# MyNiuuu/MOFA-Video

Measured on AMD Instinct MI355X. Metric: denoised frames/sec, 25f 576x1024 SVD+MOFA, 25 steps, higher is better.
Workload: dtype f16; 1 GPU; MOFA-Video-Traj, 25-frame 576x1024, 25 denoise steps + temporal VAE decode (chunk 8), single trajectory hint, SVD-XT UNet + MOFA-Adapter, CFG 1->3, seeded random weights in the reference checkpoint layout; num_frames=25, height=576, width=1024, num_inference_steps=25, decode_chunk_size=8, parallelism=1 GPU, graph_steps=False, output_finite=True

## Files before the change

### mofa_video_amd/csrc/igemm8.hip

```cpp
#include "igemm_common.h"
#include "igemm_pipe.h"

namespace {

constexpr int WM = 2, WN = 4, MI = 4, NJ = 2;
constexpr int TBM = WM * MI * 32, TBN = WN * NJ * 32;
constexpr int BKS = 64, RB = 128;
constexpr int SXB = TBM * RB, STB = SXB + TBN * RB;
constexpr int SCRATCH0 = 2 * STB, SCRATCH_WAVE = 4096;
constexpr int LDS_BYTES = SCRATCH0 + 8 * SCRATCH_WAVE;
constexpr int LOOKAHEAD_OPS = 8;

struct Cursor {
    int local;
    int ikc, ksw, ky, kx;
    int gx0, gx1;
    unsigned xo0, xo1;
    unsigned wo0, wo1, wo2, wo3;
};

template <int EPI, int VAR = 0>
__global__ __launch_bounds__(512, 2) void igemm8_f16_kernel(const mofa_igemm_args a, const int tilesN, const int ntiles,
                                                            const Aux aux) {
    constexpr bool GEGLU = (EPI & EPI_GEGLU) != 0, R1 = (EPI & EPI_R1) != 0, R2 = (EPI & EPI_R2) != 0,
                   RV = (EPI & EPI_RV) != 0;
    extern __shared__ __attribute__((aligned(16))) char smem[];
    TileWalk walk;
    walk.init(ntiles);
    if (walk.local >= walk.count) return;
    const int tid = threadIdx.x, lane = tid & 63;
    const int wave = __builtin_amdgcn_readfirstlane(tid >> 6);
    const int grp = wave >> 2;
    const int wm = wave / WN, wn = wave - wm * WN;
    const int l31 = lane & 31, lh = lane >> 5;

    const int taps = igemm_taps(a);
    const int kpt = a.Cin / BKS, nk = taps * kpt;
    const size_t Ktot = (size_t)taps * a.Cin;

    auto swz_bytes = [&](int l, int q) __attribute__((always_inline)) { return (((l & 7) ^ (4 * q + (l >> 4))) * 16); };
    auto x_row = [&](int h, int q, int hr0) __attribute__((always_inline)) { const int hr = hr0 + 8 * q; return (hr >> 6) * 128 + h * 64 + (hr & 63); };
    auto w_row = [&](int h, int q, int hr0) __attribute__((always_inline)) { const int hr = hr0 + 8 * q; return (hr >> 5) * 64 + h * 32 + (hr & 31); };
    const TapGeo tg(a);
    const BufRsrc rsx = buf_rsrc(aux.xbase, aux.x_bytes), rsw = buf_rsrc(a.w, aux.w_bytes);
    const LdsDma16 bglds16;
    auto cur_setup = [&](Cursor& c, const int h, const bool with_w) __attribute__((always_inline)) {
        const bool live = c.local < walk.count;
        const int tile = walk.start + (live ? c.local : 0);
        const int tm = fdiv(tile, aux.tiles_n), tn = tile - tm * tilesN;
        const int l = lane_now(lane), hr_l = 16 * wave + (l >> 3);
        const int g0 = pack_geo(a, aux, tm * TBM + x_row(h, 0, hr_l)), g1 = pack_geo(a, aux, tm * TBM + x_row(h, 1, hr_l));
        c.gx0 = live ? g0 : -1;
        c.gx1 = live ? g1 : -1;
        if (with_w) {
            auto w_off = [&](int hq) __attribute__((always_inline)) {
                int n = tn * TBN + w_row(hq >> 1, hq & 1, hr_l);
                n = n < a.N ? n : a.N - 1;
                const unsigned o = (unsigned)n * (unsigned)(Ktot * 2) + swz_bytes(l, hq & 1);
                return live ? o : XO_INVALID;
            };
            c.wo0 = w_off(0); c.wo1 = w_off(1); c.wo2 = w_off(2); c.wo3 = w_off(3);
        }
        c.ikc = 0; c.ksw = 0; c.ky = 0; c.kx = 0;
    };
    auto issue_x = [&](Cursor& c, const int h, const int bo) __attribute__((always_inline)) {
        if (c.ikc == 0) {
            const int l = lane_now(lane);
            c.xo0 = tap_src(a, aux, tg, c.gx0, c.ky, c.kx, swz_bytes(l, 0));
            c.xo1 = tap_src(a, aux, tg, c.gx1, c.ky, c.kx, swz_bytes(l, 1));
        }
        bglds16(rsx, c.xo0, c.ikc * (BKS * 2), smem + bo + x_row(h, 0, 16 * wave) * RB);
        bglds16(rsx, c.xo1, c.ikc * (BKS * 2), smem + bo + x_row(h, 1, 16 * wave) * RB);
    };
    auto issue_w = [&](Cursor& c, const int bo) __attribute__((always_inline)) {
        bglds16(rsw, c.wo0, c.ksw * (BKS * 2), smem + bo + SXB + w_row(0, 0, 16 * wave) * RB);
        bglds16(rsw, c.wo1, c.ksw * (BKS * 2), smem + bo + SXB + w_row(0, 1, 16 * wave) * RB);
        bglds16(rsw, c.wo2, c.ksw * (BKS * 2), smem + bo + SXB + w_row(1, 0, 16 * wave) * RB);
        bglds16(rsw, c.wo3, c.ksw * (BKS * 2), smem + bo + SXB + w_row(1, 1, 16 * wave) * RB);
    };
    auto advance = [&](Cursor& c, const int h, const bool with_w) __attribute__((always_inline)) {
        tap_advance(c, a, kpt, tg.ks);
        if (c.ksw == nk) { c.local += walk.stride; cur_setup(c, h, with_w); }
    };

    int xa[4], wa[4];
    {
        const int fsw = (l31 >> 1) & 7;
#pragma unroll
        for (int kk = 0; kk < 4; ++kk) {
            const int slot = ((kk * 2 + lh) ^ fsw) * 16;
            xa[kk] = (wm * MI * 32 + l31) * RB + slot;
            wa[kk] = SXB + (wn * NJ * 32 + l31) * RB + slot;
        }
    }

    char* scr = smem + SCRATCH0 + wave * SCRATCH_WAVE;
    const BufRsrc rsb = buf_rsrc(a.bias, a.bias ? (unsigned)a.N * 4u : 0u);
    auto bias_prefetch = [&](int nw, int slot = 0) __attribute__((always_inline)) {
        __builtin_amdgcn_raw_ptr_buffer_load_lds(rsb, (__attribute__((address_space(3))) void*)(scr + slot * 256), 4,
                                                 (unsigned)(nw + lane_now(lane)) * 4u, 0, 0, 0);
    };
    constexpr bool BIAS_INIT = GEGLU;

    Cursor ca, cb;
    ca.local = cb.local = walk.local;
    cur_setup(ca, 0, true);
    cur_setup(cb, 1, false);
    if constexpr (BIAS_INIT) {
        const int tile0 = walk.start + walk.local;
        bias_prefetch((tile0 - fdiv(tile0, aux.tiles_n) * tilesN) * TBN + wn * NJ * 32, 0);
    }
    issue_x(ca, 0, 0); issue_w(ca, 0); advance(ca, 0, true);
    issue_x(cb, 1, 0); advance(cb, 1, false);
    issue_x(ca, 0, STB); issue_w(ca, STB); advance(ca, 0, true);
    wait_vmcnt_only<LOOKAHEAD_OPS>();
    __builtin_amdgcn_s_barrier();

    f32x16 acc[MI][NJ];
    f16x8 xf[2][4], wf[2][4];
    unsigned long long tr[13] = {0, 0, 0, 0, 0, 0, 0, 0, 0, 0, 0, 0, 0}, tr_t = 0;
    if (VAR & 64) tr_t = __builtin_readcyclecounter();
    if (VAR & 32) {
#pragma unroll
        for (int kk = 0; kk < 4; ++kk) {
            xf[0][kk] = *(const f16x8*)(smem + xa[kk]);
            xf[1][kk] = *(const f16x8*)(smem + xa[kk] + 32 * RB);
            wf[0][kk] = *(const f16x8*)(smem + wa[kk]);
            wf[1][kk] = *(const f16x8*)(smem + wa[kk] + 32 * RB);
        }
    }
    auto stamp = [&](int k) __attribute__((always_inline)) {
        if (VAR & 64) { const unsigned long long t = __builtin_readcyclecounter(); tr[k] += t - tr_t; tr_t = t; }
    };
    auto phase = [&](auto pc, const int bo, const int bn) __attribute__((always_inline)) {
        constexpr int P = decltype(pc)::v;
        auto reads = [&]() __attribute__((always_inline)) {
            if (VAR & 32) return;
#pragma unroll
            for (int il = 0; il < 2; ++il)
#pragma unroll
                for (int kk = 0; kk < 4; ++kk)
                    xf[il][kk] = *(const f16x8*)(smem + xa[kk] + ((P == 2 ? 2 : 0) + il) * 32 * RB);
            if constexpr (P == 1) {
#pragma unroll
                for (int j = 0; j < 2; ++j)
#pragma unroll
                    for (int kk = 0; kk < 4; ++kk) wf[j][kk] = *(const f16x8*)(smem + wa[kk] + j * 32 * RB);
            }
        };
        auto issues = [&]() __attribute__((always_inline)) {
            if (VAR & 16) return;
            if constexpr (P == 1) issue_x(cb, 1, bn);
            if constexpr (P == 2) { issue_x(ca, 0, bo); issue_w(ca, bo); }
        };
        if (VAR & 4) { issues(); __builtin_amdgcn_sched_barrier(0); reads(); }
        else { reads(); __builtin_amdgcn_sched_barrier(0); issues(); }
        if constexpr (P == 1) advance(cb, 1, false);
        if constexpr (P == 2) advance(ca, 0, true);
        if (!(VAR & 8)) wait_vmcnt<LOOKAHEAD_OPS>(); else wait_lds();
        __builtin_amdgcn_sched_barrier(0);
        __builtin_amdgcn_s_barrier();
        __builtin_amdgcn_sched_barrier(0);
        stamp(3 * (P - 1));
        if (!(VAR & 2)) __builtin_amdgcn_s_setprio(1);
#pragma unroll
        for (int kk = 0; kk < 4; ++kk)
#pragma unroll
            for (int il = 0; il < 2; ++il)
#pragma unroll
                for (int j = 0; j < 2; ++j) {
                    constexpr int I0 = (P == 2) ? 2 : 0;
                    acc[I0 + il][j] = __builtin_amdgcn_mfma_f32_32x32x16_f16(wf[j][kk], xf[il][kk], acc[I0 + il][j], 0, 0, 0);
                }
        if (!(VAR & 2)) __builtin_amdgcn_s_setprio(0);
        stamp(3 * (P - 1) + 1);
        __builtin_amdgcn_sched_barrier(0);
        __builtin_amdgcn_s_barrier();
        __builtin_amdgcn_sched_barrier(0);
        stamp(3 * (P - 1) + 2);
    };

    auto epilogue_light = [&](auto ac, auto un, f32x16 (&acc)[MI][NJ], const int mw, const int nw, const int idx_u) __attribute__((always_inline)) {
        constexpr bool UNI = decltype(un)::v != 0;
        constexpr bool SACC1 = GEGLU && UNI;
        const int lane_e = RV ? lane_now(lane) : lane;
        const int lane = lane_e, l31 = lane & 31, lh = lane >> 5;
        f16* out = (f16*)a.out;
        float saccv = a.s_acc;
        asm volatile("" : "+v"(saccv));
        f32x4 bv[NJ][4];
        if (!BIAS_INIT && (!RV || UNI)) {
#pragma unroll
            for (int j = 0; j < NJ; ++j)
#pragma unroll
                for (int g = 0; g < 4; ++g) bv[j][g] = *(const f32x4*)(scr + (32 * j + 8 * g + 4 * lh) * 4);
        }
        const int nout = GEGLU ? a.N / 2 : a.N;
        int rv_div = a.rv_div, rv_mod_in = a.rv_mod_in, rv_mod_out = a.rv_mod_out;
        asm volatile("" : "+s"(rv_div), "+s"(rv_mod_in), "+s"(rv_mod_out));
        f32x4 rv[NJ][4];
        auto rv_load = [&](int i, f32x4 (&rv)[NJ][4]) __attribute__((always_inline)) {
            int m = mw + 32 * i + l31;
            m = m < a.M ? m : a.M - 1;
            const int idx = UNI ? idx_u : ((m / rv_div) * a.rv_mul + (m % rv_mod_in)) % rv_mod_out;
            const float* rvp = a.rowvec + (size_t)idx * a.N;
#pragma unroll
            for (int j = 0; j < NJ; ++j)
#pragma unroll
                for (int g = 0; g < 4; ++g) {
                    int n = nw + 32 * j + 8 * g + 4 * lh;
                    n = n + 4 <= a.N ? n : 0;
                    rv[j][g] = *(const f32x4*)(rvp + n);
                    if (!UNI && a.bias) rv[j][g] += *(const f32x4*)(a.bias + n);
                }
        };
        if (RV) rv_load(0, rv);
        if (RV && UNI) {
#pragma unroll
            for (int j = 0; j < NJ; ++j)
#pragma unroll
                for (int g = 0; g < 4; ++g) bv[j][g] += rv[j][g];
        }
        auto store_pair = [&](f16x4 g0, f16x4 g1, int m, int n0) __attribute__((always_inline)) {
            typedef unsigned u32x2 __attribute__((ext_vector_type(2)));
            typedef unsigned u32x4 __attribute__((ext_vector_type(4)));
            u32x2 a2 = __builtin_bit_cast(u32x2, g0), b2 = __builtin_bit_cast(u32x2, g1);
            const auto rx = __builtin_amdgcn_permlane32_swap(a2[0], b2[0], false, false);
            const auto ry = __builtin_amdgcn_permlane32_swap(a2[1], b2[1], false, false);
            const u32x4 v = {rx[0], ry[0], rx[1], ry[1]};
            const int n = n0 + 8 * lh;
            if (m < a.M && n + 8 <= nout) *(u32x4*)(out + (size_t)m * a.ldo + n) = v;
        };
#pragma unroll
        for (int i = 0; i < MI; ++i) {
            const int m = mw + 32 * i + l31;
            if constexpr (GEGLU) {
                f16x4 o[4];
#pragma unroll
                for (int g = 0; g < 4; ++g)
#pragma unroll
                    for (int e = 0; e < 4; ++e) {
                        const float val = acc[i][g >> 1][4 * (g & 1) + e];
                        const float gate = acc[i][g >> 1][8 + 4 * (g & 1) + e];
                        if constexpr (SACC1) o[g][e] = (f16)(val * (gate * gelu_phi_f(gate)));
                        else o[g][e] = (f16)(saccv * val * gelu_erf_f(saccv * gate));
                    }
                store_pair(o[0], o[1], m, nw / 2);
                store_pair(o[2], o[3], m, nw / 2 + 16);
            } else {
#pragma unroll
                for (int j = 0; j < NJ; ++j)
#pragma unroll
                    for (int g = 0; g < 4; ++g) {
                        f16x4 o;
#pragma unroll
                        for (int e = 0; e < 4; ++e) {
                            const float v = acc[i][j][4 * g + e] + (RV && !UNI ? rv[j][g][e] : bv[j][g][e]);
                            o[e] = (f16)act_apply(ac, saccv * v);
                        }
                        *(f16x4*)(scr + h16_off(l31 * 128, l31, 8 * j + 2 * g + lh)) = o;
                    }
                if (RV && !UNI && i + 1 < MI) rv_load(i + 1, rv);
#pragma unroll
                for (int p = 0; p < 4; ++p) {
                    const H16Piece r = h16_row<4 * NJ>(scr, RowLines128{}, lane, p);
                    const int mr = mw + 32 * i + r.row, n = nw + 8 * r.blk;
                    if (mr < a.M && n + 8 <= nout) *(f16x8*)(out + (size_t)mr * a.ldo + n) = r.v;
                }
            }
        }
    };
    auto epilogue_residual = [&](auto un, f32x16 (&acc)[MI][NJ], const int mw, const int nw, const int idx_u) __attribute__((always_inline)) {
        constexpr bool UNI = decltype(un)::v != 0;
        constexpr int STEPS = MI * NJ;
        constexpr int REGS = (R1 ? 8 : 0) + (R2 ? 8 : 0) + (RV && !UNI ? 16 : 0);
        constexpr int D0 = REGS <= 8 ? 8 : (REGS <= 16 ? 4 : (REGS <= 24 ? 2 : 1));
        constexpr int D = RV && UNI ? (REGS <= 8 ? 4 : 2) : (RV ? 1 : D0);
        const int lane_e = RV ? lane_now(lane) : lane;
        const int lane = lane_e, l31 = lane & 31, lh = lane >> 5;
        f16* out = (f16*)a.out;
        const f16* r1 = (const f16*)a.r1;
        const f16* r2 = (const f16*)a.r2;
        float s1v = a.s1, s2v = a.s2, saccv = a.s_acc;
        asm volatile("" : "+v"(s1v), "+v"(s2v), "+v"(saccv));
        int rv_div = a.rv_div, rv_mod_in = a.rv_mod_in, rv_mod_out = a.rv_mod_out;
        asm volatile("" : "+s"(rv_div), "+s"(rv_mod_in), "+s"(rv_mod_out));
        const int piece = lane & 3;
        struct StepLoads { f16x8 t1[2], t2[2]; f32x4 rv0[2], rv1[2]; };
        StepLoads L[D];
        auto step_loads = [&](int st, StepLoads& l) __attribute__((always_inline)) {
            const int i = st / NJ, j = st % NJ;
            const int n = nw + 32 * j + 8 * piece;
            const int nc = n + 8 <= a.N ? n : 0;
#pragma unroll
            for (int p = 0; p < 2; ++p) {
                int m = mw + 32 * i + 16 * p + (lane >> 2);
                m = m < a.M ? m : a.M - 1;
                if (R1) l.t1[p] = *(const f16x8*)(r1 + (size_t)m * a.ldr1 + nc);
                if (R2) l.t2[p] = *(const f16x8*)(r2 + (size_t)m * a.ldr2 + nc);
                if (RV && !UNI) {
                    const int idx = ((m / rv_div) * a.rv_mul + (m % rv_mod_in)) % rv_mod_out;
                    const float* q = a.rowvec + (size_t)idx * a.N + nc;
                    l.rv0[p] = *(const f32x4*)q;
                    l.rv1[p] = *(const f32x4*)(q + 4);
                }
            }
        };
        f32x4 rvu[NJ][2];
        if (RV && UNI) {
#pragma unroll
            for (int j = 0; j < NJ; ++j) {
                const int n = nw + 32 * j + 8 * piece;
                const float* q = a.rowvec + (size_t)idx_u * a.N + (n + 8 <= a.N ? n : 0);
                rvu[j][0] = *(const f32x4*)q;
                rvu[j][1] = *(const f32x4*)(q + 4);
            }
        }
#pragma unroll
        for (int st = 0; st < D && st < STEPS; ++st) step_loads(st, L[st]);
        f32x4 bv[NJ][2];
#pragma unroll
        for (int j = 0; j < NJ; ++j) {
            bv[j][0] = *(const f32x4*)(scr + (32 * j + 8 * piece) * 4);
            bv[j][1] = *(const f32x4*)(scr + (32 * j + 8 * piece + 4) * 4);
            if (RV && UNI) { bv[j][0] += rvu[j][0]; bv[j][1] += rvu[j][1]; }
        }
#pragma unroll
        for (int st = 0; st < STEPS; ++st) {
            const int i = st / NJ, j = st % NJ;
            StepLoads& l = L[st % D];
#pragma unroll
            for (int g = 0; g < 4; ++g) {
                f32x4 v;
#pragma unroll
                for (int e = 0; e < 4; ++e) v[e] = acc[i][j][4 * g + e];
                *(f32x4*)(scr + f32_off(l31 * 128, l31, 2 * g + lh)) = v;
            }
            const int n = nw + 32 * j + 8 * piece;
#pragma unroll
            for (int p = 0; p < 2; ++p) {
                const int row = 16 * p + (lane >> 2);
                const f32x4 v0 = *(const f32x4*)(scr + f32_off(row * 128, row, 2 * piece));
                const f32x4 v1 = *(const f32x4*)(scr + f32_off(row * 128, row, 2 * piece + 1));
                f16x8 o;
#pragma unroll
                for (int e = 0; e < 4; ++e) {
                    float x0 = v0[e] + bv[j][0][e], x1 = v1[e] + bv[j][1][e];
                    if (RV && !UNI) { x0 += l.rv0[p][e]; x1 += l.rv1[p][e]; }
                    x0 *= saccv; x1 *= saccv;
                    if (R1 || R2) { x0 = (float)(f16)x0; x1 = (float)(f16)x1; }
                    if (R1) { x0 += s1v * (float)l.t1[p][e]; x1 += s1v * (float)l.t1[p][4 + e]; }
                    if (R2) { x0 += s2v * (float)l.t2[p][e]; x1 += s2v * (float)l.t2[p][4 + e]; }
                    o[e] = (f16)x0; o[4 + e] = (f16)x1;
                }
                const int m = mw + 32 * i + row;
                if (m < a.M && n + 8 <= a.N) *(f16x8*)(out + (size_t)m * a.ldo + n) = o;
            }
            if (st + D < STEPS) step_loads(st + D, L[st % D]);
        }
    };

    int gt = 0;
    int bslot = 0;
    for (int cl = walk.local; cl < walk.count; cl += walk.stride, bslot ^= 1) {
        const int tile = walk.start + cl;
        const int tm = fdiv(tile, aux.tiles_n), tn = tile - tm * tilesN;
        if (VAR & 64) { stamp(9); tr[12] += nk; }
        if constexpr (BIAS_INIT) {
            int tn2 = tn;
            if (cl + walk.stride < walk.count) {
                const int tile2 = walk.start + cl + walk.stride;
                tn2 = tile2 - fdiv(tile2, aux.tiles_n) * tilesN;
            }
            bias_prefetch(tn2 * TBN + wn * NJ * 32, bslot ^ 1);
            const int lh_e = lane_now(lane) >> 5;
#pragma unroll
            for (int j = 0; j < NJ; ++j)
#pragma unroll
                for (int g = 0; g < 4; ++g) {
                    const f32x4 b = *(const f32x4*)(scr + bslot * 256 + (32 * j + 8 * g + 4 * lh_e) * 4);
#pragma unroll
                    for (int i = 0; i < MI; ++i)
#pragma unroll
                        for (int e = 0; e < 4; ++e) acc[i][j][4 * g + e] = b[e];
                }
        } else {
#pragma unroll
            for (int i = 0; i < MI; ++i)
#pragma unroll
                for (int j = 0; j < NJ; ++j)
#pragma unroll
                    for (int r = 0; r < 16; ++r) acc[i][j][r] = 0.0f;

            bias_prefetch(tn * TBN + wn * NJ * 32);
        }
        if (!(VAR & 1) && grp == 1) __builtin_amdgcn_s_barrier();
        for (int kt = 0; kt < nk; ++kt, ++gt) {
            const int bo = (gt & 1) * STB, bn = STB - bo;
            phase(IC<1>{}, bo, bn);
            phase(IC<2>{}, bo, bn);
#pragma unroll
            for (int kk = 0; kk < 4; ++kk) { xa[kk] ^= STB; wa[kk] ^= STB; }
        }
        if (!(VAR & 1) && grp == 0) __builtin_amdgcn_s_barrier();
        stamp(6);

        const int mw = tm * TBM + wm * MI * 32;
        const int nw = tn * TBN + wn * NJ * 32;
        int idx_u = -1;
        if constexpr (RV) idx_u = rowvec_uniform_idx<32 * MI>(a, mw);
        if constexpr (R1 || R2) {
            if (RV && idx_u >= 0) epilogue_residual(IC<1>{}, acc, mw, nw, idx_u);
            else epilogue_residual(IC<0>{}, acc, mw, nw, 0);
        } else if constexpr (GEGLU) {
            if (a.s_acc == 1.0f) epilogue_light(IC<MOFA_ACT_NONE>{}, IC<1>{}, acc, mw, nw, 0);
            else epilogue_light(IC<MOFA_ACT_NONE>{}, IC<0>{}, acc, mw, nw, 0);
        } else if constexpr (RV) {
            if (idx_u >= 0) epilogue_light(IC<MOFA_ACT_NONE>{}, IC<1>{}, acc, mw, nw, idx_u);
            else epilogue_light(IC<MOFA_ACT_NONE>{}, IC<0>{}, acc, mw, nw, 0);
        } else {
            if (a.act == MOFA_ACT_NONE) epilogue_light(IC<MOFA_ACT_NONE>{}, IC<0>{}, acc, mw, nw, 0);
            else if (a.act == MOFA_ACT_SILU) epilogue_light(IC<MOFA_ACT_SILU>{}, IC<0>{}, acc, mw, nw, 0);
            else if (a.act == MOFA_ACT_RELU) epilogue_light(IC<MOFA_ACT_RELU>{}, IC<0>{}, acc, mw, nw, 0);
            else epilogue_light(IC<MOFA_ACT_GELU>{}, IC<0>{}, acc, mw, nw, 0);
        }
        if (VAR & 64) { stamp(7); tr[8] += 1; }
    }
    wait_vmcnt_only<0>();
    if ((VAR & 64) && aux.trace && (tid & 255) == 0) {
#pragma unroll
        for (int k = 0; k < 13; ++k) aux.trace[((size_t)blockIdx.x * 2 + grp) * 16 + k] = tr[k];
    }
}

typedef void (*igemm8_kern_t)(const mofa_igemm_args, const int, const int, const Aux);

}

static const igemm8_kern_t k_igemm8[9] = {igemm8_f16_kernel<0>, igemm8_f16_kernel<1>, igemm8_f16_kernel<2>,
                                           igemm8_f16_kernel<3>, igemm8_f16_kernel<4>, igemm8_f16_kernel<5>,
                                           igemm8_f16_kernel<6>, igemm8_f16_kernel<7>, igemm8_f16_kernel<8>};


#ifdef MOFA_PROBE
static int s_probe_var = 0;
static unsigned long long* s_probe_trace = nullptr;
static const int k_probe_vars[] = {1, 2, 4, 8, 16, 32, 48, 64};
static const igemm8_kern_t k_trace_kern[9] = {nullptr, igemm8_f16_kernel<1, 64>, nullptr, nullptr, igemm8_f16_kernel<4, 64>, nullptr, nullptr,
                                               nullptr, igemm8_f16_kernel<8, 64>};
static const igemm8_kern_t k_probe_kern[] = {
    igemm8_f16_kernel<0, 1>, igemm8_f16_kernel<0, 2>, igemm8_f16_kernel<0, 4>, igemm8_f16_kernel<0, 8>,
    igemm8_f16_kernel<0, 16>, igemm8_f16_kernel<0, 32>, igemm8_f16_kernel<0, 48>, igemm8_f16_kernel<0, 64>};
extern "C" int mofa_igemm8_set_probe(int var, void* trace) {
    s_probe_var = var;
    s_probe_trace = (unsigned long long*)trace;
    return 0;
}
#endif

int igemm8_init() {
    if (mofa_lds_optin(k_igemm8, LDS_BYTES) != MOFA_OK) return MOFA_ELAUNCH;
#ifdef MOFA_PROBE
    if (mofa_lds_optin(k_probe_kern, LDS_BYTES) != MOFA_OK || mofa_lds_optin(k_trace_kern, LDS_BYTES) != MOFA_OK) return MOFA_ELAUNCH;
#endif
    return MOFA_OK;
}

int igemm8_launch(const mofa_igemm_args* a, int kind, int n_cu, hipStream_t stream) {
    const int taps = igemm_taps(*a);
    if (!igemm_pipe_eligible(a, kind, (long long)taps * a->Cin)) return 1;
    const int tilesM = cdiv(a->M, TBM), tilesN = cdiv(a->N, TBN);
    const long long nt = (long long)tilesM * tilesN;
    if (nt > 0x7fffffffLL) return MOFA_EINVAL;
    Aux aux = igemm_pipe_aux(a, taps, tilesN);
    igemm8_kern_t kern = k_igemm8[kind];
#ifdef MOFA_PROBE
    aux.trace = s_probe_trace;
    if (kind == 0 && s_probe_var)
        for (size_t i = 0; i < sizeof(k_probe_vars) / sizeof(int); ++i)
            if (k_probe_vars[i] == s_probe_var) kern = k_probe_kern[i];
    if (s_probe_var == 64 && k_trace_kern[kind]) kern = k_trace_kern[kind];
#endif
    hipLaunchKernelGGL(kern, dim3(igemm_grid(nt, n_cu)), dim3(512), LDS_BYTES, stream, *a, tilesN, (int)nt, aux);
    MOFA_CHECK_LAUNCH();
    return MOFA_OK;
}
```

Baseline: 4.251 frames/s.

## Switch igemm8 inner MFMA from 32x32x16 to 16x16x32 with epilogue permute

Replaces each 32x32x16 MFMA with four 16x16x32 MFMAs per accumulator tile. It also reworks the LDS fragment addressing and swizzle so each lane reads 16-row fragments over two k-halves. After the K loop, permlane16_swap shuffles the accumulators back into the 32x32 register layout the existing epilogues expect, and the bias initialisation is adapted to match. The aim is higher MFMA throughput or lower issue latency with the smaller instruction. In exchange the MFMA instruction count rises, and extra per-element vector shuffles are added around each MFMA and in the epilogue.

```diff
diff --git a/mofa_video_amd/csrc/igemm8.hip b/mofa_video_amd/csrc/igemm8.hip
--- a/mofa_video_amd/csrc/igemm8.hip
+++ b/mofa_video_amd/csrc/igemm8.hip
@@ -83,14 +83,14 @@
         if (c.ksw == nk) { c.local += walk.stride; cur_setup(c, h, with_w); }
     };
 
-    int xa[4], wa[4];
+    int xa[2], wa[2];
     {
-        const int fsw = (l31 >> 1) & 7;
-#pragma unroll
-        for (int kk = 0; kk < 4; ++kk) {
-            const int slot = ((kk * 2 + lh) ^ fsw) * 16;
-            xa[kk] = (wm * MI * 32 + l31) * RB + slot;
-            wa[kk] = SXB + (wn * NJ * 32 + l31) * RB + slot;
+        const int r = lane & 15, c = lane >> 4;
+        const int rw = 8 * ((r >> 2) & 1) + 4 * (r >> 3) + (r & 3);
+#pragma unroll
+        for (int ks = 0; ks < 2; ++ks) {
+            xa[ks] = (wm * MI * 32 + r) * RB + ((4 * ks + c) ^ ((r >> 1) & 7)) * 16;
+            wa[ks] = SXB + (wn * NJ * 32 + rw) * RB + ((4 * ks + c) ^ ((rw >> 1) & 7)) * 16;
         }
     }
 
@@ -122,12 +122,12 @@
     if (VAR & 64) tr_t = __builtin_readcyclecounter();
     if (VAR & 32) {
 #pragma unroll
-        for (int kk = 0; kk < 4; ++kk) {
-            xf[0][kk] = *(const f16x8*)(smem + xa[kk]);
-            xf[1][kk] = *(const f16x8*)(smem + xa[kk] + 32 * RB);
-            wf[0][kk] = *(const f16x8*)(smem + wa[kk]);
-            wf[1][kk] = *(const f16x8*)(smem + wa[kk] + 32 * RB);
-        }
+        for (int ks = 0; ks < 2; ++ks)
+#pragma unroll
+            for (int f = 0; f < 4; ++f) {
+                xf[ks][f] = *(const f16x8*)(smem + xa[ks] + f * 16 * RB);
+                wf[ks][f] = *(const f16x8*)(smem + wa[ks] + f * 16 * RB);
+            }
     }
     auto stamp = [&](int k) __attribute__((always_inline)) {
         if (VAR & 64) { const unsigned long long t = __builtin_readcyclecounter(); tr[k] += t - tr_t; tr_t = t; }
@@ -137,15 +137,15 @@
         auto reads = [&]() __attribute__((always_inline)) {
             if (VAR & 32) return;
 #pragma unroll
-            for (int il = 0; il < 2; ++il)
-#pragma unroll
-                for (int kk = 0; kk < 4; ++kk)
-                    xf[il][kk] = *(const f16x8*)(smem + xa[kk] + ((P == 2 ? 2 : 0) + il) * 32 * RB);
+            for (int ks = 0; ks < 2; ++ks)
+#pragma unroll
+                for (int f = 0; f < 4; ++f)
+                    xf[ks][f] = *(const f16x8*)(smem + xa[ks] + ((P == 2 ? 4 : 0) + f) * 16 * RB);
             if constexpr (P == 1) {
 #pragma unroll
-                for (int j = 0; j < 2; ++j)
-#pragma unroll
-                    for (int kk = 0; kk < 4; ++kk) wf[j][kk] = *(const f16x8*)(smem + wa[kk] + j * 32 * RB);
+                for (int ks = 0; ks < 2; ++ks)
+#pragma unroll
+                    for (int f = 0; f < 4; ++f) wf[ks][f] = *(const f16x8*)(smem + wa[ks] + f * 16 * RB);
             }
         };
         auto issues = [&]() __attribute__((always_inline)) {
@@ -164,20 +164,49 @@
         stamp(3 * (P - 1));
         if (!(VAR & 2)) __builtin_amdgcn_s_setprio(1);
 #pragma unroll
-        for (int kk = 0; kk < 4; ++kk)
+        for (int ks = 0; ks < 2; ++ks)
 #pragma unroll
             for (int il = 0; il < 2; ++il)
 #pragma unroll
-                for (int j = 0; j < 2; ++j) {
-                    constexpr int I0 = (P == 2) ? 2 : 0;
-                    acc[I0 + il][j] = __builtin_amdgcn_mfma_f32_32x32x16_f16(wf[j][kk], xf[il][kk], acc[I0 + il][j], 0, 0, 0);
-                }
+                for (int j = 0; j < 2; ++j)
+#pragma unroll
+                    for (int q = 0; q < 4; ++q) {
+                        constexpr int I0 = (P == 2) ? 2 : 0;
+                        f32x16& ab = acc[I0 + il][j];
+                        f32x4 c = {ab[4 * q], ab[4 * q + 1], ab[4 * q + 2], ab[4 * q + 3]};
+                        c = __builtin_amdgcn_mfma_f32_16x16x32_f16(wf[ks][2 * j + (q >> 1)], xf[ks][2 * il + (q & 1)], c, 0, 0, 0);
+#pragma unroll
+                        for (int e = 0; e < 4; ++e) ab[4 * q + e] = c[e];
+                    }
         if (!(VAR & 2)) __builtin_amdgcn_s_setprio(0);
         stamp(3 * (P - 1) + 1);
         __builtin_amdgcn_sched_barrier(0);
         __builtin_amdgcn_s_barrier();
         __builtin_amdgcn_sched_barrier(0);
         stamp(3 * (P - 1) + 2);
+    };
+
+    auto to_layout32 = [&](f32x16 (&acc)[MI][NJ]) __attribute__((always_inline)) {
+#pragma unroll
+        for (int i = 0; i < MI; ++i)
+#pragma unroll
+            for (int j = 0; j < NJ; ++j)
+#pragma unroll
+                for (int v = 0; v < 2; ++v)
+#pragma unroll
+                    for (int s = 0; s < 4; ++s) {
+                        const float lo = acc[i][j][8 * v + s], hi = acc[i][j][8 * v + 4 + s];
+                        const auto sw = __builtin_amdgcn_permlane16_swap(__builtin_bit_cast(unsigned, lo), __builtin_bit_cast(unsigned, hi), false, false);
+                        const unsigned slo = sw[0], shi = sw[1];
+                        acc[i][j][8 * v + s] = __builtin_bit_cast(float, slo);
+                        acc[i][j][8 * v + 4 + s] = __builtin_bit_cast(float, shi);
+                    }
+    };
+    auto pin_tuples = [&](f32x16 (&acc)[MI][NJ]) __attribute__((always_inline)) {
+#pragma unroll
+        for (int i = 0; i < MI; ++i)
+#pragma unroll
+            for (int j = 0; j < NJ; ++j) asm volatile("" : "+v"(acc[i][j]));
     };
 
     auto epilogue_light = [&](auto ac, auto un, f32x16 (&acc)[MI][NJ], const int mw, const int nw, const int idx_u) __attribute__((always_inline)) {
@@ -373,16 +402,17 @@
                 tn2 = tile2 - fdiv(tile2, aux.tiles_n) * tilesN;
             }
             bias_prefetch(tn2 * TBN + wn * NJ * 32, bslot ^ 1);
-            const int lh_e = lane_now(lane) >> 5;
+            const int lane_e = lane_now(lane);
+            const int col_e = 8 * ((lane_e >> 4) & 1) + 4 * (lane_e >> 5);
 #pragma unroll
             for (int j = 0; j < NJ; ++j)
 #pragma unroll
-                for (int g = 0; g < 4; ++g) {
-                    const f32x4 b = *(const f32x4*)(scr + bslot * 256 + (32 * j + 8 * g + 4 * lh_e) * 4);
+                for (int v = 0; v < 2; ++v) {
+                    const f32x4 b = *(const f32x4*)(scr + bslot * 256 + (32 * j + 16 * v + col_e) * 4);
 #pragma unroll
                     for (int i = 0; i < MI; ++i)
 #pragma unroll
-                        for (int e = 0; e < 4; ++e) acc[i][j][4 * g + e] = b[e];
+                        for (int e = 0; e < 4; ++e) { acc[i][j][8 * v + e] = b[e]; acc[i][j][8 * v + 4 + e] = b[e]; }
                 }
         } else {
 #pragma unroll
@@ -400,10 +430,13 @@
             phase(IC<1>{}, bo, bn);
             phase(IC<2>{}, bo, bn);
 #pragma unroll
-            for (int kk = 0; kk < 4; ++kk) { xa[kk] ^= STB; wa[kk] ^= STB; }
+            for (int ks = 0; ks < 2; ++ks) { xa[ks] ^= STB; wa[ks] ^= STB; }
         }
         if (!(VAR & 1) && grp == 0) __builtin_amdgcn_s_barrier();
         stamp(6);
+        pin_tuples(acc);
+        to_layout32(acc);
+        pin_tuples(acc);
 
         const int mw = tm * TBM + wm * MI * 32;
         const int nw = tn * TBN + wn * NJ * 32;
```

Result: no change. 4.277 frames/s, median of 6 (+0.6%).
